# fbreitwieser/krakenuniq

Measured on AMD Instinct MI355X. Metric: Mreads/s (150 bp), higher is better.
Workload: dtype u64

## Files before the change

krakenuniq_amd/csrc/ku_short.hip:

```cpp
#include <cstdlib>
#include <type_traits>

#include "ku_device.h"

#define KS_WAVES 4
#ifndef KS_KCT_LOG2
#define KS_KCT_LOG2 8
#endif
#define KS_PAD 16
#ifdef KU_ABLATION
#define KS_ABL(bit) ((ablate & (bit)) != 0)
#else
#define KS_ABL(bit) false
#endif

template <int ITEMS> struct KsGeom {
  static constexpr int MAXN = 64 * ITEMS;
  static constexpr int NWORDS = (MAXN + 31 + 15) / 16 + 3;
  static constexpr int NCODES = (MAXN + 64) / 16 + 4;
  static constexpr int NAMB = (NWORDS + 1) / 2 + 2;
  static constexpr int NMM = MAXN + 64 + 32;
  static constexpr int TCAP_LOG2 = ITEMS <= 2 ? 8 : (ITEMS <= 4 ? 9 : 10);
  static constexpr int KCT_LOG2 = KS_KCT_LOG2;
  static constexpr int RCT_LOG2 = 6;
};

__device__ __forceinline__ void ks_wave_sync() {
  __builtin_amdgcn_fence(__ATOMIC_RELEASE, "wavefront");
  __builtin_amdgcn_wave_barrier();
  __builtin_amdgcn_fence(__ATOMIC_ACQUIRE, "wavefront");
}

template <int LOG2>
__device__ __forceinline__ void ks_ct_flush(uint32_t *key, uint32_t *cnt, uint32_t *used, unsigned long long *global,
                                            uint32_t lane, uint32_t *hot = nullptr) {
  ks_wave_sync();
  for (uint32_t i = lane; i < (1u << LOG2); i += 64) {
    uint32_t kk = key[i];
#ifdef KS_DIAG_NOHOT
    if (kk == 1) kk = 0;
#endif
    if (hot && kk == 1) { *hot = cnt[i]; kk = 0; }
    if (kk) atomicAdd(&global[kk - 1], (unsigned long long)cnt[i]);
    key[i] = 0;
    cnt[i] = 0;
  }
  if (lane == 0) *used = 0;
  ks_wave_sync();
}

#define KS_RCT_SLOT 0x40000000u
__device__ __forceinline__ uint32_t ks_rct_node(uint32_t id, const KuTaxDev &tax) {
  return (id & KS_RCT_SLOT) ? ((id & ~KS_RCT_SLOT) ? tax.slot_node[id & ~KS_RCT_SLOT] : 0u) : id;
}
template <int LOG2>
__device__ __forceinline__ void ks_rct_add(uint32_t *key, uint32_t *cnt, uint32_t *used, uint32_t id, const KuTaxDev &tax,
                                           unsigned long long *global) {
  uint32_t h = (id * 2654435761u) >> (32 - LOG2);
#pragma unroll 1
  for (int probe = 0; probe < 8; ++probe) {
    uint32_t cur = key[h];
    if (cur == 0) { key[h] = id + 1; *used += 1; cur = id + 1; }
    if (cur == id + 1) { cnt[h] += 1; return; }
    h = (h + 1) & ((1u << LOG2) - 1);
  }
  atomicAdd(&global[ks_rct_node(id, tax)], 1ull);
}
template <int LOG2>
__device__ __forceinline__ void ks_rct_flush(uint32_t *key, uint32_t *cnt, uint32_t *used, const KuTaxDev &tax,
                                             unsigned long long *global, uint32_t lane, uint32_t *hot = nullptr) {
  ks_wave_sync();
  for (uint32_t i = lane; i < (1u << LOG2); i += 64) {
    uint32_t kk = key[i];
#ifdef KS_DIAG_NOHOT
    if (kk - 1 == KS_RCT_SLOT) kk = 0;
#endif
    if (hot && kk - 1 == KS_RCT_SLOT) { *hot = cnt[i]; kk = 0; }
    if (kk) atomicAdd(&global[ks_rct_node(kk - 1, tax)], (unsigned long long)cnt[i]);
    key[i] = 0;
    cnt[i] = 0;
  }
  if (lane == 0) *used = 0;
  ks_wave_sync();
}

template <int LOG2, bool TRACK>
__device__ __forceinline__ void ks_tab_add(uint32_t *t_key, uint32_t *t_cnt, uint32_t *n_distinct, uint32_t slot, uint32_t count) {
  uint32_t h = (slot * 2654435761u) >> (32 - LOG2);
  for (;;) {
    uint32_t cur = __hip_atomic_load(&t_key[h], __ATOMIC_RELAXED, __HIP_MEMORY_SCOPE_WORKGROUP);
    if (cur == 0) {
      uint32_t old = atomicCAS(&t_key[h], 0u, slot + 1);
      if (TRACK && old == 0) atomicAdd(n_distinct, 1u);
      cur = old == 0 ? slot + 1 : old;
    }
    if (cur == slot + 1) {
      atomicAdd(&t_cnt[h], count);
      break;
    }
    h = (h + 1) & ((1u << LOG2) - 1);
  }
}

template <int LOG2>
__device__ __forceinline__ uint32_t ks_tab_resolve(uint32_t *t_key, uint32_t *t_cnt, uint16_t *t_list, uint32_t *list_len,
                                                   const KuTaxDev &tax, uint32_t lane, uint32_t *urow = nullptr) {
  constexpr uint32_t TCAP = 1u << LOG2;
  if (lane == 0) *list_len = 0;
  ks_wave_sync();
  for (uint32_t i = lane; i < TCAP; i += 64)
    if (t_key[i]) t_list[atomicAdd(list_len, 1u)] = (uint16_t)i;
  ks_wave_sync();
  const uint32_t n_list = *list_len;
  uint32_t my_max = 0;
  for (uint32_t e = lane; e < n_list; e += 64) {
    const uint32_t pos = t_list[e];
    const uint32_t sl = t_key[pos] - 1;
    if (urow) atomicAdd(&urow[sl], t_cnt[pos] & 0xffffu);
    uint32_t score = 0;
    for (uint32_t i = tax.slot_anc_off[sl], i_end = tax.slot_anc_off[sl + 1]; i < i_end; ++i) {
      const uint32_t s = tax.slot_anc[i];
      uint32_t h = (s * 2654435761u) >> (32 - LOG2);
      for (;;) {
        const uint32_t cur = t_key[h];
        if (cur == s + 1) { score += t_cnt[h] & 0xffffu; break; }
        if (cur == 0) break;
        h = (h + 1) & (TCAP - 1);
      }
    }
    atomicAdd(&t_cnt[pos], score << 16);
    my_max = max(my_max, score);
  }
  my_max = ku_wave_max_u32(my_max);
  ks_wave_sync();
  uint32_t last = 0, res = 0;
  bool firstt = true;
  for (;;) {
    uint32_t my_min = 0xFFFFFFFFu;
    for (uint32_t e = lane; e < n_list; e += 64) {
      const uint32_t pos = t_list[e];
      const uint32_t s = t_key[pos] - 1;
      if ((t_cnt[pos] >> 16) == my_max && s > last) my_min = min(my_min, s);
    }
    my_min = ku_wave_min_u32(my_min);
    if (my_min == 0xFFFFFFFFu) break;
    const uint32_t node = tax.slot_node[my_min];
    res = firstt ? node : ku_lca_nodes(tax.node_parent, res, node);
    firstt = false;
    last = my_min;
  }
  ks_wave_sync();
  for (uint32_t e = lane; e < n_list; e += 64) {
    const uint32_t pos = t_list[e];
    t_key[pos] = 0;
    t_cnt[pos] = 0;
  }
  ks_wave_sync();
  return res;
}

__device__ __forceinline__ uint32_t ks_gload(const uint32_t *p) {
  return __hip_atomic_load(p, __ATOMIC_RELAXED, __HIP_MEMORY_SCOPE_AGENT);
}
__device__ __noinline__ void ks_spill_add(uint32_t *g_key, uint32_t *g_cnt, uint32_t mask, uint32_t slot, uint32_t count) {
  uint32_t h = (slot * 2654435761u) & mask;
  for (;;) {
    uint32_t cur = ks_gload(&g_key[h]);
    if (cur == 0) {
      uint32_t old = atomicCAS(&g_key[h], 0u, slot + 1);
      cur = old == 0 ? slot + 1 : old;
    }
    if (cur == slot + 1) {
      atomicAdd(&g_cnt[h], count);
      break;
    }
    h = (h + 1) & mask;
  }
}
__device__ __noinline__ void ks_spill_migrate(uint32_t *t_key, uint32_t *t_cnt, uint32_t tcap, uint32_t *g_key, uint32_t *g_cnt,
                                              uint32_t mask, bool wipe, uint32_t lane) {
  if (wipe) {
    for (uint32_t i = lane; i <= mask; i += 64) { g_key[i] = 0; g_cnt[i] = 0; }
    __threadfence();
  }
  ks_wave_sync();
  for (uint32_t i = lane; i < tcap; i += 64) {
    const uint32_t kk = t_key[i];
    if (kk) {
      ks_spill_add(g_key, g_cnt, mask, kk - 1, t_cnt[i] & 0xffffu);
      t_key[i] = 0;
      t_cnt[i] = 0;
    }
  }
  ks_wave_sync();
}
__device__ __noinline__ uint32_t ks_spill_resolve(uint32_t *g_key, uint32_t *g_cnt, uint32_t mask, const uint32_t *slot_anc_off,
                                                  const uint32_t *slot_anc, const uint32_t *slot_node, const uint32_t *node_parent,
                                                  uint32_t lane) {
  __threadfence();
  uint32_t my_max = 0;
  for (uint32_t pos = lane; pos <= mask; pos += 64) {
    const uint32_t kk = ks_gload(&g_key[pos]);
    if (!kk) continue;
    uint32_t score = 0;
    for (uint32_t i = slot_anc_off[kk - 1], i_end = slot_anc_off[kk]; i < i_end; ++i) {
      const uint32_t s = slot_anc[i];
      uint32_t h = (s * 2654435761u) & mask;
      for (;;) {
        const uint32_t cur = ks_gload(&g_key[h]);
        if (cur == s + 1) { score += ks_gload(&g_cnt[h]) & 0xffffu; break; }
        if (cur == 0) break;
        h = (h + 1) & mask;
      }
    }
    atomicAdd(&g_cnt[pos], score << 16);
    my_max = max(my_max, score);
  }
  my_max = ku_wave_max_u32(my_max);
  __threadfence();
  uint32_t last = 0, res = 0;
  bool firstt = true;
  for (;;) {
    uint32_t my_min = 0xFFFFFFFFu;
    for (uint32_t pos = lane; pos <= mask; pos += 64) {
      const uint32_t kk = ks_gload(&g_key[pos]);
      if (kk && (ks_gload(&g_cnt[pos]) >> 16) == my_max && kk - 1 > last) my_min = min(my_min, kk - 1);
    }
    my_min = ku_wave_min_u32(my_min);
    if (my_min == 0xFFFFFFFFu) break;
    const uint32_t node = slot_node[my_min];
    res = firstt ? node : ku_lca_nodes(node_parent, res, node);
    firstt = false;
    last = my_min;
  }
  for (uint32_t pos = lane; pos <= mask; pos += 64)
    if (ks_gload(&g_key[pos])) { g_key[pos] = 0; g_cnt[pos] = 0; }
  __threadfence();
  return res;
}

template <int ITEMS>
__device__ __forceinline__ uint32_t ks_g_insert_items(unsigned long long *g_key, uint64_t g_mask, const uint32_t (&slot)[ITEMS],
                                                      const uint64_t (&hash)[ITEMS], const bool (&want)[ITEMS], uint32_t *err) {
  unsigned long long key[ITEMS], old[ITEMS];
  uint64_t h[ITEMS];
#pragma unroll
  for (int j = 0; j < ITEMS; ++j) {
    key[j] = ((unsigned long long)(slot[j] + 1) << 32) | ks_encode(hash[j]);
    h[j] = ks_mix(key[j]) & g_mask;
  }
#pragma unroll
  for (int j = 0; j < ITEMS; ++j) old[j] = want[j] ? atomicCAS(&g_key[h[j]], 0ull, key[j]) : key[j];
  uint32_t fresh_n = 0;
#pragma unroll
  for (int j = 0; j < ITEMS; ++j) {
    bool fresh = want[j] && old[j] == 0ull;
    if (want[j] && old[j] != 0ull && old[j] != key[j]) {
      bool placed = false;
      for (uint32_t probe = 1; probe < 4096 && !placed; ++probe) {
        h[j] = (h[j] + 1) & g_mask;
        const unsigned long long o = atomicCAS(&g_key[h[j]], 0ull, key[j]);
        fresh = o == 0ull;
        placed = o == 0ull || o == key[j];
      }
      if (!placed) atomicOr(err, 4u);
    }
    fresh_n += (uint32_t)__popcll(__ballot(fresh));
  }
  return fresh_n;
}

#ifndef KS_OCC2
#define KS_OCC2 6
#endif
#define KS_OCC(ITEMS) ((ITEMS) == 2 ? KS_OCC2 : 4)
template <int ITEMS, bool DO_COUNTS, int KK, int MM, bool WIN, int OUT, bool ROUTE = false>
__global__ __launch_bounds__(64 * KS_WAVES, KS_OCC(ITEMS)) void ku_classify_short_kernel(
    KuDbDev db, KuTaxDev tax, KuCountsDev cnt, const uint8_t *__restrict__ seqs, uint64_t n_bytes,
    const uint64_t *__restrict__ seq_off, const uint32_t *__restrict__ seq_len, uint64_t n_reads,
    uint32_t *__restrict__ calls, uint32_t *__restrict__ taxa, uint32_t ablate, uint32_t *__restrict__ spill,
    uint32_t spill_cap, KuRunsOut ro, KuSparseFast sf, KuRouteIn rin) {
  using G = KsGeom<ITEMS>;
  constexpr uint32_t TCAP = 1u << G::TCAP_LOG2;
  __shared__ uint32_t s_codes[KS_WAVES][G::NCODES];
  __shared__ uint32_t s_amb[KS_WAVES][G::NAMB];
  __shared__ uint32_t s_mm[KS_WAVES][G::NMM];
  __shared__ uint32_t s_tkey[KS_WAVES][TCAP];
  __shared__ uint32_t s_tcnt[KS_WAVES][TCAP];
  __shared__ uint16_t s_tlist[KS_WAVES][WIN ? (int)TCAP : G::MAXN];
  __shared__ uint32_t s_kk[KS_WAVES][1 << G::KCT_LOG2], s_kc[KS_WAVES][1 << G::KCT_LOG2];
  __shared__ uint32_t s_rk[KS_WAVES][1 << G::RCT_LOG2], s_rc[KS_WAVES][1 << G::RCT_LOG2];
  __shared__ uint32_t s_misc[KS_WAVES][4];

  const uint32_t lane = threadIdx.x & 63u;
  const uint32_t wv = (uint32_t)__builtin_amdgcn_readfirstlane((int)(threadIdx.x >> 6));
  uint32_t *codes = s_codes[wv], *amb = s_amb[wv], *mmv = s_mm[wv];
  uint32_t *t_key = s_tkey[wv], *t_cnt = s_tcnt[wv];
  uint16_t *t_list = s_tlist[wv];
  uint16_t *amb16 = reinterpret_cast<uint16_t *>(amb);
  uint32_t *misc = s_misc[wv];
  const uint32_t k = KK ? (uint32_t)KK : db.k, m = KK ? (uint32_t)MM : db.nt, w = k - m + 1;
  const uint32_t key_shift = ku_key_shift(m);
  const uint32_t *tab = reinterpret_cast<const uint32_t *>(db.table);

  for (uint32_t i = lane; i < TCAP; i += 64) { t_key[i] = 0; t_cnt[i] = 0; }
  if (!ROUTE)
    for (uint32_t i = lane; i < (1u << G::KCT_LOG2); i += 64) { s_kk[wv][i] = 0; s_kc[wv][i] = 0; }
  for (uint32_t i = lane; i < (1u << G::RCT_LOG2); i += 64) { s_rk[wv][i] = 0; s_rc[wv][i] = 0; }
  if (lane < 4) misc[lane] = 0;
  ks_wave_sync();

  const uint64_t n_waves = (uint64_t)gridDim.x * KS_WAVES;
#ifdef KS_STAGGER
  {
    const uint32_t steps = ablate >> 16;
    const uint32_t slot = ((uint32_t)blockIdx.x / 256u) % 6u;
    for (uint32_t i = 0; i < slot * steps; ++i) __builtin_amdgcn_s_sleep(1);
  }
#endif
  uint32_t *g_key = WIN ? spill + ((uint64_t)blockIdx.x * KS_WAVES + wv) * 2ull * spill_cap : nullptr;
  uint32_t *g_cnt = WIN ? g_key + spill_cap : nullptr;
  bool spill_used = false;
  unsigned long long ch_pos = 0, ch_end = 0;
  if (OUT != 0 && ro.pre_base1) {
    ch_pos = ((unsigned long long)(ro.pre_base1 - 1u) + (unsigned long long)blockIdx.x * KS_WAVES + wv) * ro.chunk;
    ch_end = ch_pos + ro.chunk;
  }
  auto runs_room = [&](uint32_t need, uint32_t keep, unsigned long long &keep_base) {
    if (ch_pos + need <= ch_end) return;
    const uint32_t want_min = keep ? 2u * (keep + need) : need;
    const uint32_t want = want_min > ro.chunk ? want_min : ro.chunk;
    unsigned long long b = 0;
    if (lane == 0) b = atomicAdd(ro.counter, (unsigned long long)want);
    b = ((unsigned long long)(uint32_t)__builtin_amdgcn_readfirstlane((int)(uint32_t)(b >> 32)) << 32) |
        (uint32_t)__builtin_amdgcn_readfirstlane((int)(uint32_t)b);
    if (keep) {
      __threadfence();
      for (uint32_t i = lane; i < keep; i += 64) {
        if (keep_base + i < ro.cap && b + i < ro.cap) {
          const uint32_t *src = reinterpret_cast<const uint32_t *>(ro.runs + keep_base + i);
          ro.runs[b + i] = make_uint2(ks_gload(src), ks_gload(src + 1));
        }
      }
      keep_base = b;
    }
    ch_pos = b + keep;
    ch_end = b + want;
  };
  uint32_t sp_fresh = 0;
#ifdef KS_PREFETCH
  constexpr bool ONE_PASS = (G::NWORDS * 4 + 63) / 64 == 1;
  uint64_t r_first = (uint64_t)blockIdx.x * KS_WAVES + wv;
  uint32_t len_n = r_first < n_reads ? seq_len[r_first] : 0;
  uint64_t off_n = r_first < n_reads ? seq_off[r_first] : 0;
  uint32_t pre0 = 0, pre1 = 0;
  bool pre_ok = false;
  auto prefetch = [&](uint32_t plen, uint64_t poff) {
    const uint32_t b0 = 4 * lane;
    const uint64_t a = poff + b0, a0 = a & ~3ull;
    pre_ok = ONE_PASS && b0 < plen && a0 + 8 <= n_bytes;
    if (pre_ok) {
      const uint32_t *q = reinterpret_cast<const uint32_t *>(seqs + a0);
      pre0 = q[0];
      pre1 = q[1];
    }
  };
  if (r_first < n_reads) prefetch(len_n, off_n);
  uint32_t len_nn = r_first + n_waves < n_reads ? seq_len[r_first + n_waves] : 0;
  uint64_t off_nn = r_first + n_waves < n_reads ? seq_off[r_first + n_waves] : 0;
#endif
#ifndef KS_PREFETCH
  uint32_t len_n = 0;
  uint64_t off_n = 0;
  {
    const uint64_t r0 = (uint64_t)blockIdx.x * KS_WAVES + wv;
    if (r0 < n_reads) { len_n = seq_len[r0]; off_n = seq_off[r0]; }
  }
#endif
  for (uint64_t r = (uint64_t)blockIdx.x * KS_WAVES + wv; r < n_reads; r += n_waves) {
#ifdef KS_PREFETCH
    const uint32_t rlen = len_n;
    const uint64_t roff = off_n;
    const uint32_t cur0 = pre0, cur1 = pre1;
    const bool cur_ok = pre_ok;
    len_n = len_nn;
    off_n = off_nn;
    if (r + n_waves < n_reads) prefetch(len_n, off_n); else pre_ok = false;
    if (r + 2 * n_waves < n_reads) { len_nn = seq_len[r + 2 * n_waves]; off_nn = seq_off[r + 2 * n_waves]; }
#else
    const uint32_t rlen = len_n;
    const uint64_t roff = off_n;
    {
      const uint64_t rn = r + n_waves;
      len_n = rn < n_reads ? seq_len[rn] : 0u;
      off_n = rn < n_reads ? seq_off[rn] : 0ull;
    }
#endif
    const uint32_t n_all = rlen >= k ? rlen - k + 1 : 0;
    uint32_t rd_first = 0, rd_cnt = 0, win0 = 0;
    bool rd_table = false, rd_spill = false;
    uint32_t call_node = 0;
    unsigned long long run_base = 0;
    uint32_t run_n = 0, run_prev = 0;
    bool run_has_prev = false;
    do {
    const uint32_t len = WIN ? min(rlen - win0, (uint32_t)G::MAXN + k - 1) : rlen;
    const uint64_t off = roff + win0;
    const uint32_t n = len >= k ? len - k + 1 : 0;
    if (DO_COUNTS) {
      if (!ROUTE && misc[0] > (1u << G::KCT_LOG2) / 2) ks_ct_flush<G::KCT_LOG2>(s_kk[wv], s_kc[wv], &misc[0], cnt.n_kmers, lane);
      if (!WIN || win0 == 0)
        if (misc[1] > (1u << G::RCT_LOG2) / 2) ks_rct_flush<G::RCT_LOG2>(s_rk[wv], s_rc[wv], &misc[1], tax, cnt.n_reads, lane);
    }
    uint32_t v[ITEMS];
    bool amb_k[ITEMS];
    uint64_t hh[ITEMS];
#pragma unroll
    for (int j = 0; j < ITEMS; ++j) { v[j] = 0; amb_k[j] = false; hh[j] = 0; }

    if (ROUTE) {
      uint32_t tk[ITEMS], kbv[ITEMS];
#pragma unroll
      for (int j = 0; j < ITEMS; ++j) {
        const uint32_t p = j * 64 + lane;
        tk[j] = p < n ? taxa[off + p] : KU_ROUTE_MISS;
      }
#pragma unroll
      for (int j = 0; j < ITEMS; ++j) {
        amb_k[j] = tk[j] == KU_AMBIG;
        kbv[j] = tk[j] < KU_ROUTE_MISS ? rin.kb[tk[j] >> 5] : 0u;
      }
#pragma unroll
      for (int j = 0; j < ITEMS; ++j) v[j] = tk[j] < KU_ROUTE_MISS ? rin.ret[(uint64_t)kbv[j] + (tk[j] & 31u)] : 0u;
    } else if (n > 0) {
#pragma unroll
      for (uint32_t pl = lane; pl < (uint32_t)((G::NWORDS * 4 + 63) / 64) * 64; pl += 64) {
        const uint32_t b0 = 4 * pl;
        uint32_t c8 = 0, a4 = 0xFu;
        if (b0 < len) {
          const uint64_t a = off + b0;
          const uint64_t a0 = a & ~3ull;
          uint32_t d;
#ifdef KS_PREFETCH
          if (cur_ok && pl == lane && win0 == 0) {
            d = __builtin_amdgcn_alignbyte(cur1, cur0, (uint32_t)(a & 3ull));
          } else
#endif
          if (a0 + 8 <= n_bytes) {
            const uint32_t *q = reinterpret_cast<const uint32_t *>(seqs + a0);
            d = __builtin_amdgcn_alignbyte(q[1], q[0], (uint32_t)(a & 3ull));
          } else {
            d = 0;
            for (uint32_t j = 0; j < 4; ++j) d |= (a + j < n_bytes ? (uint32_t)seqs[a + j] : (uint32_t)'N') << (8 * j);
          }
          ku_pack_dword(d, c8, a4);
          const uint32_t valid = len - b0;
          if (valid < 4) a4 |= (1u << (4 - valid)) - 1u;
        }
        const uint32_t q4 = pl & 3u;
        uint32_t word = c8 << (24 - 8 * q4), ab = a4 << (12 - 4 * q4);
        word |= ku_quad_xor1(word);
        ab |= ku_quad_xor1(ab);
        word |= ku_quad_xor2(word);
        ab |= ku_quad_xor2(ab);
        const uint32_t wi = pl >> 2;
        if (q4 == 0 && wi < (uint32_t)G::NWORDS) {
          codes[wi] = word;
          amb16[wi ^ 1u] = (uint16_t)ab;
        }
      }
      ks_wave_sync();

      const uint32_t P = n + w - 1;
      uint64_t canon[ITEMS];
      bool is_fwd[ITEMS], ok[ITEMS];
      uint32_t pk[ITEMS + 1], wr[ITEMS + 1];
      uint32_t tacc = 0xFFFFFFFFu;
      bool tie = false;
      if (lane < KS_PAD) mmv[P + lane] = (0x03FFFFFFu - lane) << KU_PK_KEYSHIFT;
      const bool tail_round = P > (uint32_t)ITEMS * 64u;
      pk[ITEMS] = 0;
      wr[ITEMS] = (uint32_t)G::NMM - 1u;
#pragma unroll
      for (int j = 0; j <= ITEMS; ++j) {
        if (j == ITEMS && !tail_round) break;
        const uint32_t p = j * 64 + lane;
        wr[j] = p < P ? p : (uint32_t)G::NMM - 1u;
        const uint32_t wi = p >> 4, sh = (p & 15u) * 2;
        const uint32_t c0 = codes[wi], c1 = codes[wi + 1], c2 = codes[wi + 2];
        const uint64_t x = ((((uint64_t)c0 << 32) | c1) << sh >> 32 << 32) | ((((uint64_t)c1 << 32) | c2) << sh >> 32);
        const uint32_t mm = (uint32_t)(x >> (64 - 2 * m));
        const uint32_t mrc = ku_revcomp32(mm, m);
        pk[j] = ku_pk_make((mm < mrc ? mm : mrc) ^ db.xor_mask, key_shift, mm <= mrc);
        if ((m & 1u) == 0) tie |= p < P && mm == mrc;
        mmv[wr[j]] = pk[j];
        if (j < ITEMS) {
          const uint64_t fwd = x >> (64 - 2 * k);
          const uint64_t rc = ku_revcomp64(fwd, k);
          is_fwd[j] = fwd <= rc;
          canon[j] = is_fwd[j] ? fwd : rc;
          const uint32_t ai = p >> 5, as = p & 31u;
          const uint64_t a = (((uint64_t)amb[ai] << 32) | amb[ai + 1]) << as;
          amb_k[j] = p < n && (a >> (64 - k)) != 0;
          ok[j] = p < n && !amb_k[j];
        }
      }
      ks_wave_sync();

      uint32_t key[ITEMS], aoff[ITEMS];
      bool plus[ITEMS];
      if (KS_ABL(64u)) {
#pragma unroll
        for (int j = 0; j < ITEMS; ++j) { key[j] = 0; aoff[j] = 0; plus[j] = true; }
      } else {
        uint32_t blk = 1;
        uint32_t tj[ITEMS + 1];
#pragma unroll
        for (int j = 0; j <= ITEMS; ++j) tj[j] = 0xFFFFFFFFu;
        auto doubling = [&](auto nr_c) {
          constexpr int NR = decltype(nr_c)::value;
#pragma unroll
          for (uint32_t sft = 0; sft < 5; ++sft) {
            const uint32_t st = 1u << sft;
            if (2 * st > w) break;
            uint32_t nb[NR];
#pragma unroll
            for (int j = 0; j < NR; ++j) nb[j] = mmv[j * 64 + lane + st] + (st << 1);
            ks_wave_sync();
#pragma unroll
            for (int j = 0; j < NR; ++j) {
              tj[j] = min(tj[j], (pk[j] ^ nb[j]) - 2u);
              pk[j] = min(pk[j], nb[j]);
              mmv[wr[j]] = pk[j];
            }
            ks_wave_sync();
            blk = 2 * st;
          }
        };
        if (tail_round) doubling(std::integral_constant<int, ITEMS + 1>{});
        else doubling(std::integral_constant<int, ITEMS>{});
        if (w > blk) {
#pragma unroll
          for (int j = 0; j < ITEMS; ++j) {
            const uint32_t nbj = mmv[j * 64 + lane + (w - blk)] + ((w - blk) << 1);
            tj[j] = min(tj[j], (pk[j] ^ nbj) - 2u);
            pk[j] = min(pk[j], nbj);
          }
        }
#pragma unroll
        for (int j = 0; j <= ITEMS; ++j) tacc = min(tacc, j * 64 + lane < P ? tj[j] : 0xFFFFFFFFu);
        tie |= tacc < (1u << KU_PK_KEYSHIFT) - 2u;
#pragma unroll
        for (int j = 0; j < ITEMS; ++j) {
          const uint32_t t = (pk[j] >> 1) & 31u;
          key[j] = pk[j] >> KU_PK_KEYSHIFT;
          aoff[j] = is_fwd[j] ? t : w - 1 - t;
          plus[j] = ((pk[j] & 1u) != 0) == is_fwd[j];
        }
        if (__any(tie)) {
          ks_wave_sync();
#pragma unroll
          for (int j = 0; j <= ITEMS; ++j) {
            const uint32_t p = j * 64 + lane;
            if (p < P) {
              const uint32_t wi = p >> 4, sh = (p & 15u) * 2;
              const uint64_t two = ((uint64_t)codes[wi] << 32) | codes[wi + 1];
              const uint32_t mm = (uint32_t)((two << sh) >> (64 - 2 * m));
              const uint32_t mrc = ku_revcomp32(mm, m);
              mmv[p] = (mm < mrc ? mm : mrc) ^ db.xor_mask;
            }
          }
          ks_wave_sync();
#pragma unroll
          for (int j = 0; j < ITEMS; ++j) {
            const uint32_t p = j * 64 + lane;
            if (ok[j]) {
              uint32_t bin;
              key[j] = ku_anchor_exact(mmv + p, w, key_shift, is_fwd[j], aoff[j], bin);
              const uint32_t q = p + (is_fwd[j] ? aoff[j] : w - 1 - aoff[j]);
              const uint32_t wi = q >> 4, sh = (q & 15u) * 2;
              const uint64_t two = ((uint64_t)codes[wi] << 32) | codes[wi + 1];
              const uint32_t mmf = (uint32_t)((two << sh) >> (64 - 2 * m));
              const uint32_t rcm = ku_revcomp32(mmf, m);
              plus[j] = is_fwd[j] ? (mmf <= rcm) : (rcm <= mmf);
            }
          }
        }
      }
      const uint32_t *lp[ITEMS];
      uint32_t tag[ITEMS], cand[ITEMS];
      bool act[ITEMS], ovf[ITEMS];
#pragma unroll
      for (int j = 0; j < ITEMS; ++j) {
        const uint64_t locus = ku_locus_assemble(canon[j], key[j], aoff[j], plus[j], k, m);
        hh[j] = ku_fmix64(canon[j]);
        const uint64_t line = ku_locus_line(locus, db.n_lines);
        lp[j] = tab + (ok[j] ? line : 0) * KU_LINE_DWORDS;
        tag[j] = ku_table_tag(hh[j]);
        act[j] = ok[j] && !KS_ABL(1u);
        if (KS_ABL(64u)) lp[j] = tab;
      }

      uint4 h4[ITEMS];
#pragma unroll
      for (int j = 0; j < ITEMS; ++j) h4[j] = *reinterpret_cast<const uint4 *>(lp[j]);
      KuPair pr[ITEMS];
      const uint32_t *ep[ITEMS];
#pragma unroll
      for (int j = 0; j < ITEMS; ++j) {
        cand[j] = ku_tag_matches(h4[j], tag[j]) & (act[j] ? 0xFFu : 0u);
        ovf[j] = act[j] && ku_line_spilled(h4[j]);
        ep[j] = lp[j] + KU_LINE_ENTRY0 + 3 * (__builtin_ctz(cand[j] | 0x100u) & 7u);
      }
#pragma unroll
      for (int j = 0; j < ITEMS; ++j) pr[j] = *reinterpret_cast<const KuPair *>(ep[j]);
      uint32_t sb[ITEMS];
      if (OUT == 2 && DO_COUNTS) {
#pragma unroll
        for (int j = 0; j < ITEMS; ++j)
          sb[j] = reinterpret_cast<const uint8_t *>(lp[j] + KU_LINE_SEEN0)[__builtin_ctz(cand[j] | 0x100u) & 7u];
      }
#pragma unroll
      for (int j = 0; j < ITEMS; ++j) {
        const bool hit = cand[j] != 0 && (((uint64_t)pr[j].key_hi << 32) | pr[j].key_lo) == canon[j];
        v[j] = hit ? pr[j].slot : 0u;
        if (OUT == 2 && DO_COUNTS) {
          if (hit && !sb[j] && !KS_ABL(128u)) ku_seen_mark(lp[j], (uint32_t)__builtin_ctz(cand[j]));
        }
        cand[j] &= cand[j] - 1;
        act[j] = !hit && (cand[j] != 0 || ovf[j]);
      }
      bool any = false;
#pragma unroll
      for (int j = 0; j < ITEMS; ++j) any |= act[j];
      while (any) {
        any = false;
        KuPair e[ITEMS];
        uint4 a4[ITEMS];
#pragma unroll
        for (int j = 0; j < ITEMS; ++j) {
          if (act[j]) {
            if (cand[j]) {
              e[j] = *reinterpret_cast<const KuPair *>(lp[j] + KU_LINE_ENTRY0 + 3 * (__builtin_ctz(cand[j])));
            } else {
              lp[j] += KU_LINE_DWORDS;
              if (lp[j] == tab + db.n_lines * KU_LINE_DWORDS) lp[j] = tab;
              a4[j] = *reinterpret_cast<const uint4 *>(lp[j]);
            }
          }
        }
#pragma unroll
        for (int j = 0; j < ITEMS; ++j) {
          if (act[j]) {
            if (cand[j]) {
              const uint32_t ei = (uint32_t)__builtin_ctz(cand[j]);
              cand[j] &= cand[j] - 1;
              if ((((uint64_t)e[j].key_hi << 32) | e[j].key_lo) == canon[j]) {
                v[j] = e[j].slot;
                act[j] = false;
                if (OUT == 2 && DO_COUNTS && !KS_ABL(128u)) ku_seen_mark(lp[j], ei);
              }
            } else {
              cand[j] = ku_tag_matches(a4[j], tag[j]);
              ovf[j] = ku_line_spilled(a4[j]);
            }
            if (act[j]) act[j] = cand[j] != 0 || ovf[j];
            any |= act[j];
          }
        }
      }

    }

    bool uni = false;
    uint32_t uni_slot = 0;
    if (!KS_ABL(32u)) {
      uint32_t mine = 0;
#pragma unroll
      for (int j = 0; j < ITEMS; ++j)
        if (mine == 0) mine = v[j];
      const unsigned long long bal = __ballot(mine != 0);
      const uint32_t first = bal ? ku_wave_bcast(mine, (uint32_t)__ffsll((long long)bal) - 1) : 0u;
      bool diff = false;
#pragma unroll
      for (int j = 0; j < ITEMS; ++j) diff |= (v[j] != 0 && v[j] != first);
      uni = !__any(diff);
      uni_slot = uni ? first : 0u;
      if (!WIN) {
        if (!uni) {
#pragma unroll
          for (int j = 0; j < ITEMS; ++j)
            if (v[j] != 0) ks_tab_add<G::TCAP_LOG2, false>(t_key, t_cnt, nullptr, v[j], 1u);
          uint32_t *urow_hits = nullptr;
          if (OUT == 2 && DO_COUNTS && !KS_ABL(512u)) urow_hits = sf.u_cnt + (size_t)(sf.unit_of[r] - sf.unit_base) * sf.n_slots;
          call_node = ks_tab_resolve<G::TCAP_LOG2>(t_key, t_cnt, t_list, &misc[2], tax, lane, urow_hits);
        }
      } else if (bal) {
        uint32_t w_hits = 0;
#pragma unroll
        for (int j = 0; j < ITEMS; ++j) w_hits += (uint32_t)__popcll(__ballot(v[j] != 0));
        if (!rd_table && !(uni && (rd_first == 0 || rd_first == first))) {
          if (rd_first && lane == 0) ks_tab_add<G::TCAP_LOG2, true>(t_key, t_cnt, &misc[3], rd_first, rd_cnt);
          rd_table = true;
        }
        if (!rd_table) {
          rd_first = first;
          rd_cnt += w_hits;
        } else {
          ks_wave_sync();
          if (!rd_spill && misc[3] > TCAP - (uint32_t)G::MAXN - 32u) {
            ks_spill_migrate(t_key, t_cnt, TCAP, g_key, g_cnt, spill_cap - 1, !spill_used, lane);
            spill_used = true;
            rd_spill = true;
          }
          if (!rd_spill) {
            if (uni) {
              if (lane == 0) ks_tab_add<G::TCAP_LOG2, true>(t_key, t_cnt, &misc[3], first, w_hits);
            } else {
#pragma unroll
              for (int j = 0; j < ITEMS; ++j)
                if (v[j] != 0) ks_tab_add<G::TCAP_LOG2, true>(t_key, t_cnt, &misc[3], v[j], 1u);
            }
          } else {
            if (uni) {
              if (lane == 0) ks_spill_add(g_key, g_cnt, spill_cap - 1, first, w_hits);
            } else {
#pragma unroll
              for (int j = 0; j < ITEMS; ++j)
                if (v[j] != 0) ks_spill_add(g_key, g_cnt, spill_cap - 1, v[j], 1u);
            }
          }
        }
      }
    }

    const uint32_t uni_code = uni && uni_slot ? tax.slot_taxid[uni_slot] : 0u;

    uint32_t n_hit = 0, n_miss = 0;
    if (DO_COUNTS && !ROUTE && n > 0) {
      uint8_t *reg[ITEMS];
      uint32_t rank[ITEMS], seen[ITEMS];
#pragma unroll
      for (int j = 0; j < ITEMS; ++j) {
        const bool okc = j * 64 + lane < n && !amb_k[j];
        reg[j] = ku_hll_locate(cnt.registers, okc ? v[j] : 0u, hh[j], rank[j]);
        seen[j] = (okc && !KS_ABL(2u)) ? (uint32_t)*reg[j] : 0xFFu;
      }
#pragma unroll
      for (int j = 0; j < ITEMS; ++j) {
        const bool okc = j * 64 + lane < n && !amb_k[j];
        ku_hll_raise(reg[j], seen[j], rank[j]);
        if (uni) {
          n_hit += (uint32_t)__popcll(__ballot(okc && v[j] != 0));
          n_miss += (uint32_t)__popcll(__ballot(okc && v[j] == 0));
        } else if (okc && !KS_ABL(4u)) {
          ku_ct_add<G::KCT_LOG2>(s_kk[wv], s_kc[wv], &misc[0], v[j], 1, cnt.n_kmers);
        }
      }
      if (uni && lane == 0 && !KS_ABL(4u)) {
        if (n_hit) ku_ct_add<G::KCT_LOG2>(s_kk[wv], s_kc[wv], &misc[0], uni_slot, n_hit, cnt.n_kmers);
        if (n_miss) ku_ct_add<G::KCT_LOG2>(s_kk[wv], s_kc[wv], &misc[0], 0u, n_miss, cnt.n_kmers);
      }
    }

    if (OUT == 2 && DO_COUNTS && n > 0) {
      uint32_t *urow = sf.u_cnt + (size_t)(sf.unit_of[r] - sf.unit_base) * sf.n_slots;
      bool any_miss;
      if (KS_ABL(512u)) {
        any_miss = false;
      } else if (uni) {
        if (lane == 0) {
          if (n_hit) atomicAdd(&urow[uni_slot], n_hit);
          if (n_miss) atomicAdd(&urow[0], n_miss);
        }
        any_miss = n_miss != 0;
      } else if (!WIN && !KS_ABL(32u)) {
        uint32_t nm = 0;
#pragma unroll
        for (int j = 0; j < ITEMS; ++j) nm += (uint32_t)__popcll(__ballot(j * 64 + lane < n && !amb_k[j] && v[j] == 0));
        if (lane == 0 && nm) atomicAdd(&urow[0], nm);
        any_miss = nm != 0;
      } else {
        unsigned long long miss_any = 0;
#pragma unroll
        for (int j = 0; j < ITEMS; ++j) {
          const bool okc = j * 64 + lane < n && !amb_k[j];
          unsigned long long todo = __ballot(okc);
          while (todo) {
            const uint32_t lead = (uint32_t)__ffsll((long long)todo) - 1u;
            const uint32_t s0 = ku_wave_bcast(v[j], lead);
            const unsigned long long same = __ballot(okc && v[j] == s0);
            if (lane == lead) atomicAdd(&urow[s0], (uint32_t)__popcll(same));
            todo &= ~same;
          }
          miss_any |= __ballot(okc && v[j] == 0);
        }
        any_miss = miss_any != 0;
      }
      if (any_miss && sf.dense[0] == 0 && !KS_ABL(256u)) {
        bool want[ITEMS];
#pragma unroll
        for (int j = 0; j < ITEMS; ++j) want[j] = j * 64 + lane < n && !amb_k[j] && v[j] == 0;
        sp_fresh += ks_g_insert_items<ITEMS>(sf.g_key, sf.g_mask, v, hh, want, sf.err);
      }
    }

    uint32_t tcode[ITEMS];
    if (uni) {
#pragma unroll
      for (int j = 0; j < ITEMS; ++j) tcode[j] = v[j] ? uni_code : 0u;
    } else {
#pragma unroll
      for (int j = 0; j < ITEMS; ++j) tcode[j] = tax.slot_taxid[v[j]];
    }
    if (OUT == 0) {
#pragma unroll
      for (int j = 0; j < ITEMS; ++j) {
        const uint32_t p = j * 64 + lane;
        if (p < n && !KS_ABL(8u)) taxa[off + p] = amb_k[j] ? KU_AMBIG : tcode[j];
      }
    } else {
      unsigned long long sm[ITEMS];
      uint32_t carry = run_prev, w_runs = 0;
#pragma unroll
      for (int j = 0; j < ITEMS; ++j) {
        tcode[j] = amb_k[j] ? KU_AMBIG : tcode[j];
        uint32_t up = ku_wave_up1(tcode[j]);
        if (lane == 0) up = carry;
        const bool first = j == 0 && lane == 0 && !run_has_prev;
        sm[j] = __ballot(j * 64 + lane < n && (tcode[j] != up || first));
        w_runs += (uint32_t)__popcll(sm[j]);
        carry = (uint32_t)__builtin_amdgcn_readlane((int)tcode[j], 63);
      }
      if (!WIN || run_n == 0) {
        unsigned long long none = 0;
        runs_room(w_runs, 0u, none);
        run_base = ch_pos;
      } else {
        runs_room(w_runs, run_n, run_base);
      }
      uint32_t before = 0;
#pragma unroll
      for (int j = 0; j < ITEMS; ++j) {
        const unsigned long long at = ch_pos + before + (uint32_t)__popcll(sm[j] & ((1ull << lane) - 1ull));
        if (((sm[j] >> lane) & 1ull) && at < ro.cap) ro.runs[at] = make_uint2(tcode[j], win0 + j * 64 + lane);
        before += (uint32_t)__popcll(sm[j]);
      }
      ch_pos += w_runs;
      run_n += w_runs;
      run_prev = carry;
      run_has_prev = true;
    }
    if (!WIN) {
      if (OUT != 0 && lane == 0) {
        ro.run_off[r] = run_base;
        ro.run_cnt[r] = run_n;
      }
      if (lane == 0) {
        calls[r] = uni ? uni_code : tax.node_taxid[call_node];
        if (DO_COUNTS) ks_rct_add<G::RCT_LOG2>(s_rk[wv], s_rc[wv], &misc[1], uni ? (KS_RCT_SLOT | uni_slot) : call_node, tax, cnt.n_reads);
      }
      ks_wave_sync();
      break;
    }
    uint32_t nxt = win0 + (uint32_t)G::MAXN;
    if (!ROUTE && nxt < n_all) {
      uint32_t last1 = 0;
      if (lane < (uint32_t)G::NAMB) {
        const uint32_t lo = 32u * lane;
        uint32_t wd = lo < len ? amb[lane] : 0u;
        if (len - lo < 32u && lo < len) wd &= ~0u << (32u - (len - lo));
        if (wd) last1 = lo + 32u - (uint32_t)__builtin_ctz(wd);
      }
      last1 = ku_wave_max_u32(last1);
      if (last1 > (uint32_t)G::MAXN) {
        const uint32_t skip_to = min(win0 + last1, n_all);
        if (OUT == 0) {
          if (nxt + lane < skip_to) taxa[roff + nxt + lane] = KU_AMBIG;
        } else if (skip_to > nxt && run_prev != KU_AMBIG) {
          runs_room(1u, run_n, run_base);
          if (lane == 0 && ch_pos < ro.cap) ro.runs[ch_pos] = make_uint2(KU_AMBIG, nxt);
          ch_pos += 1;
          run_n += 1;
          run_prev = KU_AMBIG;
        }
        nxt = skip_to;
      }
    }
    ks_wave_sync();
    win0 = nxt;
    } while (win0 < n_all);
    if (WIN) {
      uint32_t code;
      if (!rd_table) code = rd_first ? tax.slot_taxid[rd_first] : 0u;
      else {
        call_node = rd_spill ? ks_spill_resolve(g_key, g_cnt, spill_cap - 1, tax.slot_anc_off, tax.slot_anc, tax.slot_node, tax.node_parent, lane)
                             : ks_tab_resolve<G::TCAP_LOG2>(t_key, t_cnt, t_list, &misc[2], tax, lane);
        if (lane == 0) misc[3] = 0;
        code = tax.node_taxid[call_node];
      }
      if (lane == 0) {
        calls[r] = code;
        if (OUT != 0) {
          ro.run_off[r] = run_base;
          ro.run_cnt[r] = run_n;
        }
        if (DO_COUNTS) ks_rct_add<G::RCT_LOG2>(s_rk[wv], s_rc[wv], &misc[1], rd_table ? call_node : (KS_RCT_SLOT | rd_first), tax, cnt.n_reads);
      }
      ks_wave_sync();
    }
  }
#ifndef KS_DIAG_NOFLUSH
  if (DO_COUNTS) {
    __shared__ uint32_t s_hot[KS_WAVES][2];
    if (lane < 2) s_hot[wv][lane] = 0;
    if (!ROUTE) ks_ct_flush<G::KCT_LOG2>(s_kk[wv], s_kc[wv], &misc[0], cnt.n_kmers, lane, &s_hot[wv][0]);
    ks_rct_flush<G::RCT_LOG2>(s_rk[wv], s_rc[wv], &misc[1], tax, cnt.n_reads, lane, &s_hot[wv][1]);
    __syncthreads();
    if (wv == 0 && lane < 2) {
      unsigned long long sum = 0;
#pragma unroll
      for (int q = 0; q < KS_WAVES; ++q) sum += s_hot[q][lane];
      if (sum) atomicAdd(lane == 0 ? &cnt.n_kmers[0] : &cnt.n_reads[0], sum);
    }
  }
#endif
  if (OUT == 2 && lane == 0 && sp_fresh) atomicAdd(sf.g_count, (unsigned long long)sp_fresh);
}

static uint32_t ks_one_pass_max() { return getenv("KU_SHORT_ONE_PASS_MAX") ? (uint32_t)atoi(getenv("KU_SHORT_ONE_PASS_MAX")) : 192u; }
uint32_t ku_short_max_kmers(const KuDbDev &db) {
  const bool whole = db.bin_lo == 0 && db.bin_hi == (1ull << (2 * db.nt));
  return (db.table && whole) ? ks_one_pass_max() : 0;
}
uint32_t ku_short_max_kmers_windowed(const KuDbDev &db) {
  return ku_short_max_kmers(db) ? 65535u : 0u;
}

static unsigned ks_grid(uint64_t n_reads, int items, int n_cu) {
  const char *oe = getenv("KU_SHORT_BLOCKS_PER_CU");
  const uint64_t per_cu = oe ? (uint64_t)atoi(oe) : (n_reads < 500000 ? 1ull : 2ull) * KS_OCC(items);
  const uint64_t want = (n_reads + KS_WAVES - 1) / KS_WAVES, cap = (uint64_t)n_cu * per_cu;
  return (unsigned)(want < cap ? want : cap);
}
static uint32_t ks_spill_cap(uint32_t max_kmers, uint32_t n_slots) {
  const uint32_t distinct = max_kmers < n_slots ? max_kmers : n_slots;
  uint32_t cap = 1024;
  while (cap < 2 * distinct) cap <<= 1;
  return cap;
}
uint64_t ku_short_workspace_bytes(uint32_t max_kmers, uint32_t n_slots, uint64_t n_reads, int n_cu) {
  if (max_kmers <= ks_one_pass_max()) return 0;
  return (uint64_t)ks_grid(n_reads, 2, n_cu) * KS_WAVES * 2ull * ks_spill_cap(max_kmers, n_slots) * 4ull;
}

uint64_t ku_short_grid_waves(uint64_t n_reads, uint32_t max_kmers, int n_cu) {
  const bool windowed = max_kmers > ks_one_pass_max();
  return (uint64_t)ks_grid(n_reads, max_kmers <= 128 || windowed ? 2 : 3, n_cu) * KS_WAVES;
}

int ku_launch_classify_short(const KuDbDev &db, const KuTaxDev &tax, const KuCountsDev &cnt, const uint8_t *d_seqs,
                             uint64_t n_bytes, const uint64_t *d_seq_off, const uint32_t *d_seq_len, uint64_t n_reads,
                             uint32_t max_kmers, uint32_t flags, uint32_t *d_calls, uint32_t *d_taxa, uint32_t *d_hits,
                             void *d_workspace, uint64_t workspace_bytes, int n_cu, hipStream_t stream,
                             const KuRunsOut *runs_out, const KuSparseFast *sparse) {
  if (n_reads == 0) return KU_OK;
  const bool counts = !(flags & KU_F_NO_COUNTS);
  if (flags & KU_F_KEEP_SLOTS) return KU_EINVAL;
  if (sparse && (!runs_out || !counts)) return KU_EINVAL;
  if (!runs_out && !d_taxa) return KU_EINVAL;
  if (d_hits && hipMemsetAsync(d_hits, 0, n_reads * 4, stream) != hipSuccess) return KU_EHIP;
  const char *ab = getenv("KU_ABLATE");
  const uint32_t ablate = ab ? (uint32_t)atoi(ab) : 0u;
  const bool windowed = max_kmers > ks_one_pass_max();
  const int items = max_kmers <= 128 || windowed ? 2 : 3;
  const dim3 grid(ks_grid(n_reads, items, n_cu)), block(64 * KS_WAVES);
  uint32_t spill_cap = 0;
  if (windowed) {
    if (max_kmers > 65535u) return KU_EINVAL;
    spill_cap = ks_spill_cap(max_kmers, tax.n_slots);
    if (!d_workspace || workspace_bytes < (uint64_t)grid.x * KS_WAVES * 2ull * spill_cap * 4ull) return KU_EINVAL;
  }
  const KuRunsOut ro = runs_out ? *runs_out : KuRunsOut{};
  const KuSparseFast sf = sparse ? *sparse : KuSparseFast{};
  const int out = sparse ? 2 : (runs_out ? 1 : 0);
#define KS_LAUNCH(I, C, K, M, W, O)                                                                                          \
  hipLaunchKernelGGL((ku_classify_short_kernel<I, C, K, M, W, O>), grid, block, 0, stream, db, tax, cnt, d_seqs, n_bytes,    \
                     d_seq_off, d_seq_len, n_reads, d_calls, d_taxa, ablate, (uint32_t *)d_workspace, spill_cap, ro, sf, KuRouteIn{})
  const int geo = !counts || db.k != 31 ? 0 : (db.nt == 13 ? 13 : (db.nt == 15 ? 15 : 0));
#define KS_GEO(I, W, O)                                      \
  do {                                                       \
    if (!counts) KS_LAUNCH(I, false, 0, 0, W, (O) == 2 ? 1 : (O)); \
    else if (geo == 13) KS_LAUNCH(I, true, 31, 13, W, O);    \
    else if (geo == 15) KS_LAUNCH(I, true, 31, 15, W, O);    \
    else KS_LAUNCH(I, true, 0, 0, W, O);                     \
  } while (0)
#define KS_OUT(I, W)                  \
  do {                                \
    if (out == 0) KS_GEO(I, W, 0);    \
    else if (out == 1) KS_GEO(I, W, 1); \
    else KS_GEO(I, W, 2);             \
  } while (0)
  if (windowed) KS_OUT(2, true);
  else if (max_kmers <= 128) KS_OUT(2, false);
  else KS_OUT(3, false);
#undef KS_OUT
#undef KS_GEO
#undef KS_LAUNCH
  return hipGetLastError() == hipSuccess ? KU_OK : KU_EHIP;
}

uint32_t ku_route_resolve_max_kmers() { return 65535u; }
int ku_launch_route_resolve(const KuDbDev &db, const KuTaxDev &tax, const KuCountsDev &cnt, const uint64_t *d_seq_off,
                            const uint32_t *d_seq_len, uint64_t n_reads, uint32_t max_kmers, uint32_t flags, uint32_t *d_calls,
                            uint32_t *d_taxa, uint32_t *d_hits, const uint32_t *d_kb, const uint32_t *d_ret, void *d_workspace,
                            uint64_t workspace_bytes, int n_cu, hipStream_t stream, const KuRunsOut *runs_out) {
  if (n_reads == 0) return KU_OK;
  if (!d_taxa || !d_kb || !d_seq_off || !d_seq_len || !d_calls || max_kmers > 65535u) return KU_EINVAL;
  if (flags & (KU_F_KEEP_SLOTS | KU_F_QUICK)) return KU_EINVAL;
  if (d_hits && hipMemsetAsync(d_hits, 0, n_reads * 4, stream) != hipSuccess) return KU_EHIP;
  const bool counts = !(flags & KU_F_NO_COUNTS), windowed = max_kmers > 128;
  const dim3 grid(ks_grid(n_reads, 2, n_cu)), block(64 * KS_WAVES);
  uint32_t spill_cap = 0;
  if (windowed) {
    spill_cap = ks_spill_cap(max_kmers, tax.n_slots);
    if (!d_workspace || workspace_bytes < (uint64_t)grid.x * KS_WAVES * 2ull * spill_cap * 4ull) return KU_EINVAL;
  }
  const KuRunsOut ro = runs_out ? *runs_out : KuRunsOut{};
  const KuRouteIn rin{d_kb, d_ret};
#define KS_RLAUNCH(C, W, O)                                                                                                     \
  hipLaunchKernelGGL((ku_classify_short_kernel<2, C, 0, 0, W, O, true>), grid, block, 0, stream, db, tax, cnt, (const uint8_t *)nullptr, \
                     (uint64_t)0, d_seq_off, d_seq_len, n_reads, d_calls, d_taxa, 0u, (uint32_t *)d_workspace, spill_cap, ro,    \
                     KuSparseFast{}, rin)
#define KS_RSEL(W, O)                  \
  do {                                 \
    if (counts) KS_RLAUNCH(true, W, O); \
    else KS_RLAUNCH(false, W, O);      \
  } while (0)
  if (windowed) { if (runs_out) KS_RSEL(true, 1); else KS_RSEL(true, 0); }
  else { if (runs_out) KS_RSEL(false, 1); else KS_RSEL(false, 0); }
#undef KS_RSEL
#undef KS_RLAUNCH
  return hipGetLastError() == hipSuccess ? KU_OK : KU_EHIP;
}
```

Before: 553.0.

## Use 32-bit read indices, throttle count flushes, skip clean ambiguity checks, reuse revcomp

Read indices in the grid-stride loop become 32-bit, and the launchers gain a guard that rejects read counts too large for 32 bits. Count-table flush checks now run only every fourth iteration, the ambiguity mask is skipped when no lane in the wave saw an ambiguous base, and the minimizer reverse complement is taken from the k-mer reverse complement instead of being recomputed. The minimizer doubling loop now picks the tail-round width at each step and drops the -2 bias on the tie bits. Delaying flushes can let the local count tables fill beyond the half-full threshold, and the tie-bit and flush-on-window changes may alter semantics.

Result: no change. 548.0 (-0.9%).

```diff
diff --git a/krakenuniq_amd/csrc/ku_short.hip b/krakenuniq_amd/csrc/ku_short.hip
--- a/krakenuniq_amd/csrc/ku_short.hip
+++ b/krakenuniq_amd/csrc/ku_short.hip
@@ -310,7 +310,7 @@
   if (lane < 4) misc[lane] = 0;
   ks_wave_sync();
 
-  const uint64_t n_waves = (uint64_t)gridDim.x * KS_WAVES;
+  const uint32_t n_waves = gridDim.x * KS_WAVES, n_rd = (uint32_t)n_reads;
 #ifdef KS_STAGGER
   {
     const uint32_t steps = ablate >> 16;
@@ -350,9 +350,9 @@
   uint32_t sp_fresh = 0;
 #ifdef KS_PREFETCH
   constexpr bool ONE_PASS = (G::NWORDS * 4 + 63) / 64 == 1;
-  uint64_t r_first = (uint64_t)blockIdx.x * KS_WAVES + wv;
-  uint32_t len_n = r_first < n_reads ? seq_len[r_first] : 0;
-  uint64_t off_n = r_first < n_reads ? seq_off[r_first] : 0;
+  uint32_t r_first = blockIdx.x * KS_WAVES + wv;
+  uint32_t len_n = r_first < n_rd ? seq_len[r_first] : 0;
+  uint64_t off_n = r_first < n_rd ? seq_off[r_first] : 0;
   uint32_t pre0 = 0, pre1 = 0;
   bool pre_ok = false;
   auto prefetch = [&](uint32_t plen, uint64_t poff) {
@@ -365,19 +365,21 @@
       pre1 = q[1];
     }
   };
-  if (r_first < n_reads) prefetch(len_n, off_n);
-  uint32_t len_nn = r_first + n_waves < n_reads ? seq_len[r_first + n_waves] : 0;
-  uint64_t off_nn = r_first + n_waves < n_reads ? seq_off[r_first + n_waves] : 0;
+  if (r_first < n_rd) prefetch(len_n, off_n);
+  uint32_t len_nn = r_first + n_waves < n_rd ? seq_len[r_first + n_waves] : 0;
+  uint64_t off_nn = r_first + n_waves < n_rd ? seq_off[r_first + n_waves] : 0;
 #endif
 #ifndef KS_PREFETCH
   uint32_t len_n = 0;
   uint64_t off_n = 0;
   {
-    const uint64_t r0 = (uint64_t)blockIdx.x * KS_WAVES + wv;
-    if (r0 < n_reads) { len_n = seq_len[r0]; off_n = seq_off[r0]; }
+    const uint32_t r0 = blockIdx.x * KS_WAVES + wv;
+    if (r0 < n_rd) { len_n = seq_len[r0]; off_n = seq_off[r0]; }
   }
 #endif
-  for (uint64_t r = (uint64_t)blockIdx.x * KS_WAVES + wv; r < n_reads; r += n_waves) {
+  constexpr uint32_t KS_CT_EVERY = 4;
+  uint32_t ct_wait = 0;
+  for (uint32_t r = blockIdx.x * KS_WAVES + wv; r < n_rd; r += n_waves) {
 #ifdef KS_PREFETCH
     const uint32_t rlen = len_n;
     const uint64_t roff = off_n;
@@ -385,15 +387,15 @@
     const bool cur_ok = pre_ok;
     len_n = len_nn;
     off_n = off_nn;
-    if (r + n_waves < n_reads) prefetch(len_n, off_n); else pre_ok = false;
-    if (r + 2 * n_waves < n_reads) { len_nn = seq_len[r + 2 * n_waves]; off_nn = seq_off[r + 2 * n_waves]; }
+    if (r + n_waves < n_rd) prefetch(len_n, off_n); else pre_ok = false;
+    if (r + 2 * n_waves < n_rd) { len_nn = seq_len[r + 2 * n_waves]; off_nn = seq_off[r + 2 * n_waves]; }
 #else
     const uint32_t rlen = len_n;
     const uint64_t roff = off_n;
     {
-      const uint64_t rn = r + n_waves;
-      len_n = rn < n_reads ? seq_len[rn] : 0u;
-      off_n = rn < n_reads ? seq_off[rn] : 0ull;
+      const uint32_t rn = r + n_waves;
+      len_n = rn < n_rd ? seq_len[rn] : 0u;
+      off_n = rn < n_rd ? seq_off[rn] : 0ull;
     }
 #endif
     const uint32_t n_all = rlen >= k ? rlen - k + 1 : 0;
@@ -408,9 +410,12 @@
     const uint64_t off = roff + win0;
     const uint32_t n = len >= k ? len - k + 1 : 0;
     if (DO_COUNTS) {
-      if (!ROUTE && misc[0] > (1u << G::KCT_LOG2) / 2) ks_ct_flush<G::KCT_LOG2>(s_kk[wv], s_kc[wv], &misc[0], cnt.n_kmers, lane);
-      if (!WIN || win0 == 0)
+      if (ct_wait == 0) {
+        if (!ROUTE && misc[0] > (1u << G::KCT_LOG2) / 2) ks_ct_flush<G::KCT_LOG2>(s_kk[wv], s_kc[wv], &misc[0], cnt.n_kmers, lane);
         if (misc[1] > (1u << G::RCT_LOG2) / 2) ks_rct_flush<G::RCT_LOG2>(s_rk[wv], s_rc[wv], &misc[1], tax, cnt.n_reads, lane);
+        ct_wait = KS_CT_EVERY;
+      }
+      --ct_wait;
     }
     uint32_t v[ITEMS];
     bool amb_k[ITEMS];
@@ -433,6 +438,7 @@
 #pragma unroll
       for (int j = 0; j < ITEMS; ++j) v[j] = tk[j] < KU_ROUTE_MISS ? rin.ret[(uint64_t)kbv[j] + (tk[j] & 31u)] : 0u;
     } else if (n > 0) {
+      bool dirty = false;
 #pragma unroll
       for (uint32_t pl = lane; pl < (uint32_t)((G::NWORDS * 4 + 63) / 64) * 64; pl += 64) {
         const uint32_t b0 = 4 * pl;
@@ -455,6 +461,7 @@
           }
           ku_pack_dword(d, c8, a4);
           const uint32_t valid = len - b0;
+          dirty |= (a4 >> (valid < 4 ? 4 - valid : 0u)) != 0;
           if (valid < 4) a4 |= (1u << (4 - valid)) - 1u;
         }
         const uint32_t q4 = pl & 3u;
@@ -470,6 +477,7 @@
         }
       }
       ks_wave_sync();
+      const bool clean = !__any(dirty);
 
       const uint32_t P = n + w - 1;
       uint64_t canon[ITEMS];
@@ -490,15 +498,25 @@
         const uint32_t c0 = codes[wi], c1 = codes[wi + 1], c2 = codes[wi + 2];
         const uint64_t x = ((((uint64_t)c0 << 32) | c1) << sh >> 32 << 32) | ((((uint64_t)c1 << 32) | c2) << sh >> 32);
         const uint32_t mm = (uint32_t)(x >> (64 - 2 * m));
-        const uint32_t mrc = ku_revcomp32(mm, m);
-        pk[j] = ku_pk_make((mm < mrc ? mm : mrc) ^ db.xor_mask, key_shift, mm <= mrc);
-        if ((m & 1u) == 0) tie |= p < P && mm == mrc;
-        mmv[wr[j]] = pk[j];
+        uint32_t mrc;
         if (j < ITEMS) {
           const uint64_t fwd = x >> (64 - 2 * k);
           const uint64_t rc = ku_revcomp64(fwd, k);
           is_fwd[j] = fwd <= rc;
           canon[j] = is_fwd[j] ? fwd : rc;
+          ok[j] = p < n;
+          mrc = (uint32_t)rc & (uint32_t)((1ull << (2 * m)) - 1ull);
+        } else {
+          mrc = ku_revcomp32(mm, m);
+        }
+        pk[j] = ku_pk_make((mm < mrc ? mm : mrc) ^ db.xor_mask, key_shift, mm <= mrc);
+        if ((m & 1u) == 0) tie |= p < P && mm == mrc;
+        mmv[wr[j]] = pk[j];
+      }
+      if (!clean) {
+#pragma unroll
+        for (int j = 0; j < ITEMS; ++j) {
+          const uint32_t p = j * 64 + lane;
           const uint32_t ai = p >> 5, as = p & 31u;
           const uint64_t a = (((uint64_t)amb[ai] << 32) | amb[ai + 1]) << as;
           amb_k[j] = p < n && (a >> (64 - k)) != 0;
@@ -517,28 +535,28 @@
         uint32_t tj[ITEMS + 1];
 #pragma unroll
         for (int j = 0; j <= ITEMS; ++j) tj[j] = 0xFFFFFFFFu;
-        auto doubling = [&](auto nr_c) {
+        auto step = [&](auto nr_c, uint32_t st) {
           constexpr int NR = decltype(nr_c)::value;
-#pragma unroll
-          for (uint32_t sft = 0; sft < 5; ++sft) {
-            const uint32_t st = 1u << sft;
-            if (2 * st > w) break;
-            uint32_t nb[NR];
-#pragma unroll
-            for (int j = 0; j < NR; ++j) nb[j] = mmv[j * 64 + lane + st] + (st << 1);
-            ks_wave_sync();
-#pragma unroll
-            for (int j = 0; j < NR; ++j) {
-              tj[j] = min(tj[j], (pk[j] ^ nb[j]) - 2u);
-              pk[j] = min(pk[j], nb[j]);
-              mmv[wr[j]] = pk[j];
-            }
-            ks_wave_sync();
-            blk = 2 * st;
+          uint32_t nb[NR];
+#pragma unroll
+          for (int j = 0; j < NR; ++j) nb[j] = mmv[j * 64 + lane + st] + (st << 1);
+          ks_wave_sync();
+#pragma unroll
+          for (int j = 0; j < NR; ++j) {
+            tj[j] = min(tj[j], pk[j] ^ nb[j]);
+            pk[j] = min(pk[j], nb[j]);
+            mmv[wr[j]] = pk[j];
           }
+          ks_wave_sync();
         };
-        if (tail_round) doubling(std::integral_constant<int, ITEMS + 1>{});
-        else doubling(std::integral_constant<int, ITEMS>{});
+#pragma unroll
+        for (uint32_t sft = 0; sft < 5; ++sft) {
+          const uint32_t st = 1u << sft;
+          if (2 * st > w) break;
+          if (P >= (uint32_t)ITEMS * 64u + 2 * st) step(std::integral_constant<int, ITEMS + 1>{}, st);
+          else step(std::integral_constant<int, ITEMS>{}, st);
+          blk = 2 * st;
+        }
         if (w > blk) {
 #pragma unroll
           for (int j = 0; j < ITEMS; ++j) {
@@ -943,6 +961,7 @@
   const uint64_t want = (n_reads + KS_WAVES - 1) / KS_WAVES, cap = (uint64_t)n_cu * per_cu;
   return (unsigned)(want < cap ? want : cap);
 }
+#define KS_MAX_READS(blocks) (0xFFFFFFFFull - (uint64_t)(blocks) * KS_WAVES)
 static uint32_t ks_spill_cap(uint32_t max_kmers, uint32_t n_slots) {
   const uint32_t distinct = max_kmers < n_slots ? max_kmers : n_slots;
   uint32_t cap = 1024;
@@ -975,6 +994,7 @@
   const bool windowed = max_kmers > ks_one_pass_max();
   const int items = max_kmers <= 128 || windowed ? 2 : 3;
   const dim3 grid(ks_grid(n_reads, items, n_cu)), block(64 * KS_WAVES);
+  if (n_reads > KS_MAX_READS(grid.x)) return KU_EINVAL;
   uint32_t spill_cap = 0;
   if (windowed) {
     if (max_kmers > 65535u) return KU_EINVAL;
@@ -1021,6 +1041,7 @@
   if (d_hits && hipMemsetAsync(d_hits, 0, n_reads * 4, stream) != hipSuccess) return KU_EHIP;
   const bool counts = !(flags & KU_F_NO_COUNTS), windowed = max_kmers > 128;
   const dim3 grid(ks_grid(n_reads, 2, n_cu)), block(64 * KS_WAVES);
+  if (n_reads > KS_MAX_READS(grid.x)) return KU_EINVAL;
   uint32_t spill_cap = 0;
   if (windowed) {
     spill_cap = ks_spill_cap(max_kmers, tax.n_slots);
```
